# hbdat/cvpr22_cross_modal_pseudo_labeling

Hardware: AMD Instinct MI355X
Metric: images/sec student-teacher train step (COCO 800x1333) (higher is better)
Workload: dtype f32 (bf16x3 split MFMA, fp32 accum); 1 GPU; student_teacher_mask_rcnn_uncertainty.yaml R-50-C4, 2 img/GPU 3x800x1333, fwd+bwd+allreduce+SGD; global_batch=2, parallelism=dp1, losses_finite=True, pipelined=True

## Files before the change

### cvpr22_cross_modal_pseudo_labeling_amd/_C.py

```python
import contextlib
import functools
import ctypes
import threading

import torch

from . import _cpu, _lib

_L = _lib.load()


def _stream():
    return torch._C._cuda_getCurrentRawStream(torch.cuda.current_device())


class _Same:

    def __enter__(self):
        return None

    def __exit__(self, *exc):
        return False


# ... 594 lines not shown
        _lib.check(rc, "match_encode")
    return idx, lab, reg


def rpn_match_encode(gt_boxes, anchors, visibility, high_threshold, low_threshold, allow_low_quality_matches, weights):
    gt_boxes, anchors = _dev(gt_boxes, "gt_boxes"), _dev(anchors, "anchors")
    if not (visibility.is_cuda and visibility.dtype == torch.bool and visibility.shape == (anchors.shape[0],)):
        raise RuntimeError("rpn_match_encode: visibility must be a bool HIP tensor [A]")
    visibility = visibility.contiguous()
    g, a = gt_boxes.shape[0], anchors.shape[0]
    if g == 0:
        raise ValueError("No ground-truth boxes available for one of the images during training")
    labels = torch.empty((a,), dtype=torch.int64, device=anchors.device)
    reg = torch.empty((a, 4), dtype=torch.float32, device=anchors.device)
    scratch = torch.empty((g,), dtype=torch.int32, device=anchors.device)
    wx, wy, ww, wh = weights
    with _on(anchors.device):
        rc = _L.ovis_rpn_match_encode_f32(gt_boxes.data_ptr(), anchors.data_ptr(), visibility.data_ptr(), g, a, high_threshold,
                                          low_threshold, int(bool(allow_low_quality_matches)), wx, wy, ww, wh, scratch.data_ptr(),
                                          labels.data_ptr(), reg.data_ptr(), _stream())
    _lib.check(rc, "rpn_match_encode")
    return labels, reg


def project_masks(masks, gt_index, boxes, resolution):
    if not (masks.is_cuda and masks.dim() == 3 and masks.dtype in (torch.bool, torch.uint8)):
        raise RuntimeError("project_masks: [G,H,W] bool / uint8 HIP tensor expected")
    masks = masks.contiguous()
    boxes = _dev(boxes, "boxes")
    gt_index = gt_index.to(torch.int64).contiguous()
    p = boxes.shape[0]
    out = torch.empty((p, resolution, resolution), dtype=torch.float32, device=boxes.device)
    if p:
        with _on(boxes.device):
            rc = _L.ovis_project_masks_f32(masks.data_ptr(), gt_index.data_ptr(), boxes.data_ptr(), p, masks.shape[1],
                                           masks.shape[2], resolution, int(masks.dtype == torch.bool), out.data_ptr(),
                                           _stream())
        _lib.check(rc, "project_masks")
    return out


def sample_fg_bg(labels, batch_size, max_positives, seed):
    if not labels.is_cuda or labels.dtype != torch.int64 or labels.dim() != 1:
        raise RuntimeError("sample_fg_bg: 1-D int64 HIP tensor expected (the product path has no CPU fallback)")
    labels = labels.contiguous()
    sel = torch.empty((batch_size,), dtype=torch.int64, device=labels.device)
    slots = torch.empty((batch_size,), dtype=torch.int64, device=labels.device)
    counts = torch.empty((2,), dtype=torch.int32, device=labels.device)
    with _on(labels.device):
        rc = _L.ovis_sample_fg_bg(labels.data_ptr(), labels.numel(), int(batch_size), int(max_positives),
                                  int(seed) & 0xFFFFFFFFFFFFFFFF, sel.data_ptr(), slots.data_ptr(), counts.data_ptr(), _stream())
    _lib.check(rc, "sample_fg_bg")
    return sel, slots, counts


def gather_rows(index, boxes_a=None, boxes_b=None, ints_a=None, ints_b=None):
    index = _dev(index, "index", torch.int64)
    n = index.numel()
    srcs = [None if t is None else _dev(t, "boxes", torch.float32) for t in (boxes_a, boxes_b)] + \
           [None if t is None else _dev(t, "ints", torch.int64) for t in (ints_a, ints_b)]
    for t in srcs[:2]:
        if t is not None and (t.dim() != 2 or t.shape[1] != 4):
            raise RuntimeError("gather_rows: float sources must be [P, 4]")
    for t in srcs[2:]:
        if t is not None and t.dim() != 1:
            raise RuntimeError("gather_rows: int64 sources must be [P]")
    outs = [None if t is None else torch.empty((n,) + tuple(t.shape[1:]), dtype=t.dtype, device=t.device) for t in srcs]
    if n:
        with _on(index.device):
            rc = _L.ovis_gather_rows(index.data_ptr(), n, _ptr(srcs[0]), _ptr(outs[0]), _ptr(srcs[1]), _ptr(outs[1]),
                                     _ptr(srcs[2]), _ptr(outs[2]), _ptr(srcs[3]), _ptr(outs[3]), _stream())
        _lib.check(rc, "gather_rows")
    return tuple(outs)


def project_pasted_masks(mask_probs, gt_boxes, gt_index, boxes, image_size, resolution, threshold=0.5):
    mask_probs, gt_boxes, boxes = _dev(mask_probs, "mask_probs"), _dev(gt_boxes, "gt_boxes"), _dev(boxes, "boxes")
    gt_index = _dev(gt_index, "gt_index", torch.int64)
    p = boxes.shape[0]
    out = torch.empty((p, resolution, resolution), dtype=torch.float32, device=boxes.device)
    if p == 0:
        return out
    if mask_probs.dim() != 3 or mask_probs.shape[1] != mask_probs.shape[2] or gt_boxes.shape != (mask_probs.shape[0], 4):
        raise RuntimeError("project_pasted_masks: expected mask_probs [G,M,M] and gt_boxes [G,4]")
    with _on(boxes.device):
        rc = _L.ovis_project_pasted_masks_f32(mask_probs.data_ptr(), gt_boxes.data_ptr(), gt_index.data_ptr(),
                                              boxes.data_ptr(), p, int(image_size[0]), int(image_size[1]),
                                              mask_probs.shape[1], int(resolution), float(threshold), out.data_ptr(), _stream())
    _lib.check(rc, "project_pasted_masks")
    return out


def paste_masks(probs, boxes, image_size, threshold=0.5):
    probs, boxes = _dev(probs, "probs"), _dev(boxes, "boxes")
    if probs.dim() != 3 or probs.shape[1] != probs.shape[2] or boxes.shape != (probs.shape[0], 4):
        raise RuntimeError("paste_masks: expected probs [P,M,M] and boxes [P,4]")
    p, h, w = probs.shape[0], int(image_size[0]), int(image_size[1])
    out = torch.empty((p, h, w), dtype=torch.bool, device=probs.device)
    if p == 0:
        return out
    with _on(probs.device):
        rc = _L.ovis_paste_masks_u8(probs.data_ptr(), boxes.data_ptr(), p, probs.shape[1], h, w, float(threshold),
                                    out.data_ptr(), _stream())
    _lib.check(rc, "paste_masks")
    return out

# ... 1127 lines not shown
```

### cvpr22_cross_modal_pseudo_labeling_amd/csrc/targets.hip

```cpp
#include "ovis_common.h"
#define OVIS_HD __device__ __forceinline__
#include "mask_crop_geom.h"
#include "pasted_geom.h"

namespace {
__global__ __launch_bounds__(256) void match_encode_kernel(const float* __restrict__ gt, const long* __restrict__ gt_labels,
                                                          const float* __restrict__ prop, int G, int P, float high,
                                                          float low, int between_label_mode, float wx, float wy,
                                                          float ww, float wh, long* __restrict__ matched_idx,
                                                          long* __restrict__ labels, float* __restrict__ reg) {
  const int p = blockIdx.x * 256 + threadIdx.x;
  if (p >= P) return;
  const float4 b = *(const float4*)(prop + 4 * p);
  const float area_b = (b.z - b.x + 1.f) * (b.w - b.y + 1.f);
  float best = -1.f;
  int arg = 0;
  for (int g = 0; g < G; ++g) {
    const float4 a = *(const float4*)(gt + 4 * g);
    const float area_a = (a.z - a.x + 1.f) * (a.w - a.y + 1.f);
    const float w = fmaxf(fminf(a.z, b.z) - fmaxf(a.x, b.x) + 1.f, 0.f);
    const float h = fmaxf(fminf(a.w, b.w) - fmaxf(a.y, b.y) + 1.f, 0.f);
    const float inter = w * h;
    const float iou = inter / (area_a + area_b - inter);
    if (iou > best) {
// ... 333 lines not shown
    const int c = (int)(e >> 14);
    if (c == 2) return;
    if (taken(i, e, c)) {
      if (c == 1) pos_slot[pat++] = at;
      sel_idx[at++] = i;
    }
  });
  for (int j = total_sel + tid; j < batch_size; j += kSampThreads) sel_idx[j] = 0;
  for (int j = total_pos + tid; j < batch_size; j += kSampThreads) pos_slot[j] = 0;
  if (tid == 0) {
    counts[0] = total_sel;
    counts[1] = total_pos;
  }
}

__global__ __launch_bounds__(256) void project_pasted_masks_kernel(const float* __restrict__ probs,
                                                                  const float* __restrict__ gt_boxes,
                                                                  const long* __restrict__ gt_index,
                                                                  const float* __restrict__ boxes, int P, int H, int W,
                                                                  int Mp, int M, float thr, float* __restrict__ out) {
  const long i = (long)blockIdx.x * 256 + threadIdx.x;
  const long total = (long)P * M * M;
  if (i >= total) return;
  const int dx = (int)(i % M), dy = (int)((i / M) % M), p = (int)(i / ((long)M * M));
  const MaskCropWindow c = mask_crop_window(*(const float4*)(boxes + 4 * p), W, H);
  const MaskAxisTap ty = mask_axis_tap(dy, c.h, (float)M), tx = mask_axis_tap(dx, c.w, (float)M);
  const float xmin = c.xmin, ymin = c.ymin, y0 = ty.i0, y1 = ty.i1, ly = ty.lam, x0 = tx.i0, x1 = tx.i1, lx = tx.lam;
  const long g = gt_index[p];
  const float4 gb = *(const float4*)(gt_boxes + 4 * g);
  const PastedBox pb = pasted_box(gb, Mp);
  const int4 bx = pb.bx;
  const int bw = pb.bw, bh = pb.bh;
  const float* pr = probs + g * Mp * Mp;
  const int Y0 = (int)(y0 + ymin), Y1 = (int)(y1 + ymin), X0 = (int)(x0 + xmin), X1 = (int)(x1 + xmin);
  const float v00 = pasted_pixel(pr, Mp, bx, bw, bh, thr, H, W, Y0, X0), v01 = pasted_pixel(pr, Mp, bx, bw, bh, thr, H, W, Y0, X1);
  const float v10 = pasted_pixel(pr, Mp, bx, bw, bh, thr, H, W, Y1, X0), v11 = pasted_pixel(pr, Mp, bx, bw, bh, thr, H, W, Y1, X1);
  const float v = (1.f - ly) * ((1.f - lx) * v00 + lx * v01) + ly * ((1.f - lx) * v10 + lx * v11);
  out[i] = v != 0.f ? 1.f : 0.f;
}
__global__ __launch_bounds__(256) void gather_rows_kernel(const long long* __restrict__ index, int n,
                                                         const float4* __restrict__ fa, float4* __restrict__ fa_out,
                                                         const float4* __restrict__ fb, float4* __restrict__ fb_out,
                                                         const long long* __restrict__ ia, long long* __restrict__ ia_out,
                                                         const long long* __restrict__ ib, long long* __restrict__ ib_out) {
  const int i = blockIdx.x * blockDim.x + threadIdx.x;
  if (i >= n) return;
  const long long r = index[i];
  if (fa) fa_out[i] = fa[r];
  if (fb) fb_out[i] = fb[r];
  if (ia) ia_out[i] = ia[r];
  if (ib) ib_out[i] = ib[r];
}

}

extern "C" int ovis_sample_fg_bg(const int64_t* labels, int num, int batch_size, int max_positives, uint64_t seed,
                                 int64_t* selected, int64_t* positive_slots, int32_t* counts, void* stream) {
  if (num < 0 || batch_size <= 0 || max_positives < 0 || max_positives > batch_size) return OVIS_EINVAL;
  if (!selected || !positive_slots || !counts || (num > 0 && !labels)) return OVIS_EINVAL;
  constexpr int kCacheBytes = 150 * 1024;
  if (2L * num + 16 <= kCacheBytes) {
    static bool attr_set = false;
    if (!attr_set) {
      OVIS_HIP_TRY(hipFuncSetAttribute((const void*)sample_fg_bg_kernel<true>, hipFuncAttributeMaxDynamicSharedMemorySize, kCacheBytes));
      attr_set = true;
    }
    const int lds = ((2 * num + 16 + 255) / 256) * 256;
    hipLaunchKernelGGL(sample_fg_bg_kernel<true>, dim3(1), dim3(kSampThreads), lds, (hipStream_t)stream, (const long*)labels, num,
                       batch_size, max_positives, (unsigned long long)seed, (long*)selected, (long*)positive_slots, counts);
  } else {
    hipLaunchKernelGGL(sample_fg_bg_kernel<false>, dim3(1), dim3(kSampThreads), 0, (hipStream_t)stream, (const long*)labels, num,
                       batch_size, max_positives, (unsigned long long)seed, (long*)selected, (long*)positive_slots, counts);
  }
  OVIS_LAUNCH_CHECK();
  return OVIS_OK;
}

extern "C" int ovis_project_pasted_masks_f32(const float* mask_probs, const float* gt_boxes, const int64_t* gt_index,
                                             const float* boxes, int num, int image_height, int image_width,
                                             int prob_resolution, int resolution, float threshold, float* out,
                                             void* stream) {
  if (num < 0 || image_height <= 0 || image_width <= 0 || prob_resolution <= 0 || resolution <= 0) return OVIS_EINVAL;
  if (num == 0) return OVIS_OK;
  if (!mask_probs || !gt_boxes || !gt_index || !boxes || !out) return OVIS_EINVAL;
  if (((uintptr_t)boxes & 15) || ((uintptr_t)gt_boxes & 15)) return OVIS_ERANGE;
  const long total = (long)num * resolution * resolution;
  hipLaunchKernelGGL(project_pasted_masks_kernel, dim3((unsigned)((total + 255) / 256)), dim3(256), 0, (hipStream_t)stream,
                     mask_probs, gt_boxes, (const long*)gt_index, boxes, num, image_height, image_width, prob_resolution,
                     resolution, threshold, out);
  OVIS_LAUNCH_CHECK();
  return OVIS_OK;
}

extern "C" int ovis_match_encode_f32(const float* gt_boxes, const int64_t* gt_labels, const float* proposals,
                                     int num_gt, int num_proposals, float high_threshold, float low_threshold,
                                     int between_keeps_label, float wx, float wy, float ww, float wh,
                                     int64_t* matched_idx, int64_t* labels, float* regression_targets, void* stream) {
  if (num_gt <= 0 || num_proposals < 0) return OVIS_EINVAL;
  if (num_proposals == 0) return OVIS_OK;
  if (!gt_boxes || !gt_labels || !proposals || !matched_idx || !labels) return OVIS_EINVAL;
  if (((uintptr_t)gt_boxes & 15) || ((uintptr_t)proposals & 15) || ((uintptr_t)regression_targets & 15)) return OVIS_ERANGE;
  hipLaunchKernelGGL(match_encode_kernel, dim3((num_proposals + 255) / 256), dim3(256), 0, (hipStream_t)stream, gt_boxes,
                     (const long*)gt_labels, proposals, num_gt, num_proposals, high_threshold, low_threshold,
                     between_keeps_label, wx, wy, ww, wh, (long*)matched_idx, (long*)labels, regression_targets);
  OVIS_LAUNCH_CHECK();
  return OVIS_OK;
// ... 56 lines not shown
```

### cvpr22_cross_modal_pseudo_labeling_amd/engine/trainer.py

```python
import logging
import time

import torch

from . import comm
from .. import _C


def total_loss(loss_dict):
    terms = [v if torch.is_tensor(v) else torch.as_tensor(float(v)) for v in loss_dict.values()]
    if len(terms) < 3 or not all(t.is_cuda for t in terms):
        return sum(terms)
    return torch.stack([t.reshape(()) for t in terms]).sum()


class StepPolicy:

    def __init__(self, accumulation_steps=1, clip_grad_norm_at=-1.0):
        self.accumulation_steps = max(int(accumulation_steps), 1)
        self.clip_grad_norm_at = float(clip_grad_norm_at)
        self.prepare_weights_ahead = True
        self.micro = 0
        self.fresh = True

# ... 28 lines not shown


def train_step(model, optimizer, reducer, images, targets, scheduler=None, policy=None, iteration=None):
    policy = policy or _default_policy(reducer)
    loss_dict = model(images, targets)
    policy.begin(reducer)
    losses = policy.scale(total_loss(loss_dict))
    losses.backward()
    policy.end(reducer, optimizer, scheduler, iteration, model)
    return loss_dict


def _default_policy(reducer):
    pol = getattr(reducer, "_step_policy", None)
    if pol is None:
        pol = reducer._step_policy = StepPolicy()
    return pol


def _record_stream(obj, stream):
    if torch.is_tensor(obj):
        if obj.is_cuda:
            obj.record_stream(stream)
    elif isinstance(obj, dict):
        for v in obj.values():
            _record_stream(v, stream)
    elif isinstance(obj, (list, tuple)):
        for v in obj:
            _record_stream(v, stream)
    elif hasattr(obj, "device_tensors"):
        _record_stream(obj.device_tensors(), stream)


_SIDE_STREAMS = {}


def side_stream(priority):
    key = (torch.cuda.current_device(), priority)
    if key not in _SIDE_STREAMS:
        _SIDE_STREAMS[key] = torch.cuda.Stream(priority=priority)
    return _SIDE_STREAMS[key]


def branch_stream():
    return side_stream(-1)


class PipelinedTrainer:

    def __init__(self, model, optimizer, reducer, scheduler=None, threaded=True, side_priority=-1, policy=None):
        self.model, self.optimizer, self.reducer, self.scheduler = model, optimizer, reducer, scheduler
        self.policy = policy or StepPolicy()
        self.enabled = hasattr(model, "forward_frozen") and torch.cuda.is_available()
        bert = getattr(model, "bert", None)
        if self.enabled and bert is not None and any(p.requires_grad for p in bert.parameters()):
            self.enabled = False
        self.side = side_stream(side_priority) if self.enabled else None
        self.pending = None
        self.threaded = threaded
        self.worker = None
        self.worker_error = None

    def _frozen_on_side(self, images, targets, after_event, device):
        try:
            torch.cuda.set_device(device)
            with torch.cuda.stream(self.side):
                if after_event is not None:
                    self.side.wait_event(after_event)
                with _C.co_scheduled():
                    frozen = self.model.forward_frozen(images, targets)
                done = torch.cuda.Event()
                done.record(self.side)
            self.pending = ((id(images), id(targets)), frozen, done)
        except BaseException as e:
            self.worker_error = e

    def _launch_frozen(self, images, targets, after_event=None, threaded=False):
        device = torch.cuda.current_device()
        if threaded:
            import threading
            self.worker = threading.Thread(target=self._frozen_on_side, args=(images, targets, after_event, device))
            self.worker.start()
        else:
            self._frozen_on_side(images, targets, after_event, device)
            self._check_worker()

    def _check_worker(self):
        if self.worker is not None:
            self.worker.join()
            self.worker = None
        if self.worker_error is not None:
            e, self.worker_error = self.worker_error, None
            raise e

    def step(self, images, targets, next_batch=None, iteration=None):
        if not self.enabled:
            return train_step(self.model, self.optimizer, self.reducer, images, targets, self.scheduler, self.policy, iteration)
        main = torch.cuda.current_stream()
        inputs_ready = torch.cuda.Event()
        inputs_ready.record(main)
        self._check_worker()
        if self.pending is None or self.pending[0] != (id(images), id(targets)):
            self._launch_frozen(images, targets, inputs_ready)
        _, frozen, done = self.pending
        self.pending = None
        main.wait_event(done)
# ... 81 lines not shown
```

### cvpr22_cross_modal_pseudo_labeling_amd/modeling/roi_heads.py

```python
import bisect

import torch
import torch.nn.functional as F
from torch import nn

from .. import _C
from ..layers import (Conv2d, ConvTranspose2d, ROIAlign, linear_mfma, smooth_l1_loss, smooth_l1_picked, stochastic_mask_bce,
                      text_logits, weighted_cross_entropy)
from ..layers.derived import derived
from .backbone import HeadFeatures, ResNetHead
from .box_coder import BoxCoder
from .matcher import BalancedPositiveNegativeSampler, Matcher
from .structures import BoxList, PastedMasks, PolygonMasks, RleMasks, SampledBoxList, box_iou, boxlist_nms, cat_boxlist


def _cat(tensors, dim=0):
    return tensors[0] if len(tensors) == 1 else torch.cat(tensors, dim)


class Pooler(nn.Module):
    def __init__(self, output_size, scales, sampling_ratio):
        super().__init__()
        if len(scales) != 1:
            raise NotImplementedError("single-level pooler only (C4)")
        self.pooler = ROIAlign(output_size, spatial_scale=scales[0], sampling_ratio=sampling_ratio)
        self.output_size = output_size

    @staticmethod
    def convert_to_roi_format(boxes):
        if boxes and all(b.bbox.is_cuda and b.bbox.dtype == torch.float32 for b in boxes):
            return _C.rois_from_boxes([b.bbox for b in boxes])
        parts = []
        for i, b in enumerate(boxes):
            ids = torch.full((len(b), 1), float(i), dtype=b.bbox.dtype, device=b.bbox.device)
            parts.append(torch.cat([ids, b.bbox], dim=1))
        return _cat(parts, 0)

    def forward(self, x, boxes):
        return self.pooler(x[0], self.convert_to_roi_format(boxes))

    def forward_strided_nhwc(self, x, boxes, bin_stride):
        return self.pooler.forward_strided_nhwc(x[0], self.convert_to_roi_format(boxes), bin_stride)


class ResNet50Conv5ROIFeatureExtractor(nn.Module):
    def __init__(self, cfg, head_cfg):
        super().__init__()
        res = head_cfg.POOLER_RESOLUTION
        self.pooler = Pooler((res, res), head_cfg.POOLER_SCALES, head_cfg.POOLER_SAMPLING_RATIO)
        self.head = ResNetHead(cfg)
        self.out_channels = self.head.out_channels

    def forward(self, x, proposals, pooled_only=False):
        return self.forward_rois(x, self.pooler.convert_to_roi_format(proposals), pooled_only=pooled_only)

    def forward_rois(self, x, rois, select=None, pooled_only=False):
        p = self.pooler.pooler
        s = self.head.pooler_stride() if x[0].is_cuda else 0
        if s:
            need_grad = torch.is_grad_enabled() and x[0].requires_grad
            if not need_grad and x[0].shape[1] % 32 == 0 and self.head.pooled_pair_ok():
                ph, pw = p.output_size
                yp, (oh, ow) = _C.roi_align_forward_strided_pair(x[0], rois, p.spatial_scale, ph, pw, p.sampling_ratio, s)
                return self.head.forward_pooled_nhwc(None, yp, (rois.shape[0], oh, ow), select=select, pooled_only=pooled_only)
            return self.head.forward_pooled_nhwc(p.forward_strided_nhwc(x[0], rois, s), select=select, pooled_only=pooled_only)
        return HeadFeatures(self.head(p(x[0], rois)))


class FastRCNNPredictor(nn.Module):

# ... 36 lines not shown
        first = self.emb_pred if self.embedding_based else self.cls_score
        n1 = first.out_features
        n = n1 + self.bbox_pred.out_features
        pad = (-n) % 128 if x.is_cuda else 0

        def concatenated():
            zw, zb = self._zero_rows(pad, x)
            return (torch.cat([first.weight, self.bbox_pred.weight] + ([zw] if pad else []), 0),
                    torch.cat([first.bias, self.bbox_pred.bias] + ([zb] if pad else []), 0))
        w, b = derived((first.weight, first.bias, self.bbox_pred.weight, self.bbox_pred.bias), ("predictor", pad), concatenated)
        y = linear_mfma(x, w, b)
        head, bbox = y[:, :n1], y[:, n1:n]
        if not self.embedding_based:
            return head, bbox
        cls_logit = text_logits(head, self.cls_score if cls_embs is None else cls_embs.to(head.device))
        return cls_logit, bbox

    def _zero_rows(self, pad, x):
        z = getattr(self, "_zero_pad", None)
        if pad and (z is None or z[0].shape[0] != pad or z[0].device != x.device):
            z = (x.new_zeros((pad, self.bbox_pred.in_features)), x.new_zeros((pad,)))
            self._zero_pad = z
        return z if pad else (None, None)

    def embed(self, x):
        if not self.embedding_based:
            raise RuntimeError("FastRCNNPredictor.embed: MODEL.ROI_BOX_HEAD.EMBEDDING_BASED is False -- there is no embedding "
                               "projection to align with text")
        return linear_mfma(self.pooled(x), self.emb_pred.weight, self.emb_pred.bias)

    def set_class_embeddings(self, embs):
        if not self.embedding_based:
            raise RuntimeError("set_class_embeddings: MODEL.ROI_BOX_HEAD.EMBEDDING_BASED is False -- the classifier is a "
                               "learned Linear over NUM_CLASSES")
        self.num_classes = embs.shape[0]
        self.cls_score = embs.to(self.emb_pred.weight.device)


class FastRCNNLossComputation:
    def __init__(self, cfg):
        rh = cfg.MODEL.ROI_HEADS
        self.matcher = Matcher(rh.FG_IOU_THRESHOLD, rh.BG_IOU_THRESHOLD, allow_low_quality_matches=False)
        self.sampler = BalancedPositiveNegativeSampler(rh.BATCH_SIZE_PER_IMAGE, rh.POSITIVE_FRACTION)
        self.box_coder = BoxCoder(weights=rh.BBOX_REG_WEIGHTS)
        self.cls_agnostic_bbox_reg = cfg.MODEL.CLS_AGNOSTIC_BBOX_REG
        self.bg_weight = cfg.MODEL.ROI_BOX_HEAD.LOSS_WEIGHT_BACKGROUND
        self.generator = None
        self.device_sampler = True

    def subsample(self, proposals, targets):
        return self.subsample_many([(proposals, targets)])[0]

    def subsample_many(self, groups):
        if not all(p.bbox.is_cuda for props, _ in groups for p in props) or self.matcher.allow_low_quality_matches \
                or not self.device_sampler:
            return [self._subsample_tensor_ops(props, tgts) for props, tgts in groups]
        pending = []
        for props, tgts in groups:
            for prop, tgt in zip(props, tgts):
                idx, labels, reg = _C.match_encode(tgt.bbox, tgt.get_field("labels"), prop.bbox, self.matcher.high_threshold,
                                                   self.matcher.low_threshold, self.box_coder.weights)
                sel, slots, counts = self.sampler.sample_device(labels, self.generator)
                pending.append((prop, idx, labels, reg, sel, slots, counts))
        cnt = torch.stack([p[-1] for p in pending]).tolist() if pending else []
        out, k = [], 0
        for props, _ in groups:
            group = []
            for _p in props:
                prop, idx, labels, reg, sel, slots, _c = pending[k]
                n, npos = cnt[k]
                k += 1
                bbox_s, reg_s, labels_s, idx_s = _C.gather_rows(sel[:n], prop.bbox, reg, labels, idx)
                b = BoxList(bbox_s, prop.size)
                b.add_field("labels", labels_s)
                b.add_field("regression_targets", reg_s)
                b.add_field("matched_gt", idx_s)
                group.append(SampledBoxList(b, slots[:npos]))
            out.append(group)
        self._proposals = out[-1]
        return out

    def _subsample_tensor_ops(self, proposals, targets):
        out = []
        labels_all = []
        for prop, tgt in zip(proposals, targets):
            if prop.bbox.is_cuda and not self.matcher.allow_low_quality_matches:
                idx, labels, reg = _C.match_encode(tgt.bbox, tgt.get_field("labels"), prop.bbox,
                                                   self.matcher.high_threshold, self.matcher.low_threshold,
                                                   self.box_coder.weights)
            else:
                matched = self.matcher(box_iou(tgt.bbox, prop.bbox))
                idx = matched.clamp(min=0)
                labels = tgt.get_field("labels")[idx].to(torch.int64)
                labels[matched == Matcher.BELOW_LOW_THRESHOLD] = 0
                labels[matched == Matcher.BETWEEN_THRESHOLDS] = -1
                reg = self.box_coder.encode(tgt.bbox[idx], prop.bbox)
            prop.add_field("labels", labels)
            prop.add_field("regression_targets", reg)
            prop.add_field("matched_gt", idx)
            labels_all.append(labels)
        pos, neg = self.sampler(labels_all, generator=self.generator)
        for prop, p, n in zip(proposals, pos, neg):
            out.append(SampledBoxList(prop[torch.nonzero(p | n).squeeze(1)]))
        self._proposals = out
        return out

    def __call__(self, class_logits, box_regression, proposals=None):
        if proposals is None:
            proposals = self._proposals
        labels = _cat([p.get_field("labels") for p in proposals], 0)
        reg_targets = _cat([p.get_field("regression_targets") for p in proposals], 0)
        pos = positives_index(proposals)
        if pos is None:
            pos = torch.nonzero(labels > 0).squeeze(1)
        if box_regression.is_cuda and labels.numel():
            box_loss = smooth_l1_picked(box_regression, reg_targets, pos, None if self.cls_agnostic_bbox_reg else labels, 4,
                                        1.0, labels.numel())
        else:
            if self.cls_agnostic_bbox_reg:
                picked = box_regression.index_select(0, pos)[:, 4:8]
            else:
                map_inds = 4 * labels[pos][:, None] + torch.tensor([0, 1, 2, 3], device=class_logits.device)
                picked = box_regression[pos[:, None], map_inds]
            box_loss = smooth_l1_loss(picked, reg_targets.index_select(0, pos), size_average=False, beta=1) / labels.numel()
        cls_loss = weighted_cross_entropy(class_logits, labels, self.bg_weight)
        return cls_loss, box_loss


def positives_index(proposals):
    parts, off = [], 0
    for p in proposals:
        if not isinstance(p, SampledBoxList) or p.pos_index is None:
            return None
# ... 479 lines not shown
        self.avg_uncertain = "N/A"

    def forward(self, features, proposals, targets=None, compute_uncertain=False, eps=None):
        if self.training:
            sel = positives_index(proposals)
            if sel is not None:
                proposals = [positive_proposals(p) for p in proposals]
            else:
                positive_inds = [p.get_field("labels") > 0 for p in proposals]
                proposals = [p[i] for p, i in zip(proposals, positive_inds)]
                sel = _cat(positive_inds, 0)
        if self.training and self.share:
            fl = features.permute(0, 2, 3, 1) if features.dim() == 4 else None
            if fl is not None and fl.is_contiguous() and not features.is_contiguous():
                x = fl[sel].permute(0, 3, 1, 2)
            else:
                x = features[sel]
        else:
            x = self.feature_extractor(features, proposals).maps
        if self.training:
            return x, proposals, dict(loss_mask=self.fused_training_loss(x, proposals, targets, compute_uncertain, eps))
        if compute_uncertain:
            mask_logits, scale = self.predictor(x, True, eps=eps)
            self.log, self.avg_uncertain = scale.max(), scale.mean()
        else:
            mask_logits = self.predictor(x)
        prob = mask_logits.sigmoid()
        if self.cls_agnostic_mask:
            prob = prob[:, 1][:, None]
        else:
            labels = _cat([b.get_field("labels") for b in proposals], 0)
            prob = prob[torch.arange(prob.shape[0], device=prob.device), labels][:, None]
        results = []
        for p, b in zip(prob.split([len(b) for b in proposals], 0), proposals):
            out = b.copy_with_fields(b.fields())
            out.add_field("mask", p if self.masker is None else self.masker(p, b))
            results.append(out)
        return x, results, {}

    def fused_training_loss(self, x, proposals, targets, compute_uncertain=False, eps=None):
        mu, sigma = self.predictor.forward_parts(x)
        if compute_uncertain and sigma is not None:
            self.log, self.avg_uncertain = sigma.max(), sigma.mean()
            if eps is None:
                eps = torch.randn((1, *mu.shape), device=mu.device, dtype=mu.dtype)
            else:
                eps = eps[:, : mu.shape[0]].to(mu.device)
            return self.loss_evaluator.fused(proposals, mu, sigma, eps, targets)
        return self.loss_evaluator.fused(proposals, mu, None, None, targets)


class CombinedROIHeads(nn.ModuleDict):
    batch_branches = True

    def __init__(self, cfg, in_channels, is_teacher=False):
        heads = [("box", ROIBoxHead(cfg, in_channels, is_teacher))]
        if cfg.MODEL.MASK_ON:
            heads.append(("mask", ROIMaskHead(cfg, in_channels)))
        super().__init__(heads)
        self.cfg = cfg
        self.mask_on = cfg.MODEL.MASK_ON
        if self.mask_on and cfg.MODEL.ROI_MASK_HEAD.SHARE_BOX_FEATURE_EXTRACTOR:
            self.mask.feature_extractor = self.box.feature_extractor

    def branches_batchable(self, feat):
        return (self.training and feat.is_cuda and (not self.mask_on or (self.mask.share and self.mask.cls_agnostic_mask))
                and self.batch_branches)

    def forward_branches(self, feat, branches):
        box = self.box
        with torch.no_grad():
            sampled = box.loss_evaluator.subsample_many([(br["proposals"], br["targets"]) for br in branches])
        rois = _C.rois_from_boxes([p.bbox for props in sampled for p in props],
                                  [img for br in branches for img in br["image_ids"]])
        sel_pos = positives_index([p for props in sampled for p in props]) if self.mask_on else None
        x, pooled, handed = box.feature_extractor.forward_rois([feat], rois, select=sel_pos)
        pooled = box.predictor.pooled(pooled if pooled is not None else x)
        counts = [sum(len(p) for p in props) for props in sampled]
        out, off = [], 0
        for br, props, cnt in zip(branches, sampled, counts):
            class_logits, box_regression = box.predictor(pooled[off:off + cnt], br["cls_embs"])
            lc, lb = box.loss_evaluator(class_logits, box_regression, props)
            out.append(dict(loss_classifier=lc, loss_box_reg=lb))
            off += cnt
        if self.mask_on:
            mask = self.mask
            sel = sel_pos
            if sel is not None:
                pos_all = [[positive_proposals(p) for p in props] for props in sampled]
            else:
                pos_masks = [[p.get_field("labels") > 0 for p in props] for props in sampled]
                sel = _cat([m for ms in pos_masks for m in ms], 0)
                pos_all = [[p[m] for p, m in zip(props, ms)] for props, ms in zip(sampled, pos_masks)]
            fl = x.permute(0, 2, 3, 1)
            if handed is not None and handed[0] is sel:
                xs = handed[1].view(sel.numel(), x.shape[2], x.shape[3], x.shape[1]).permute(0, 3, 1, 2)
            else:
                xs = fl[sel].permute(0, 3, 1, 2) if (fl.is_contiguous() and not x.is_contiguous()) else x[sel]
            off = 0
            for br, pos_props, losses in zip(branches, pos_all, out):
                k = sum(len(p) for p in pos_props)
                losses["loss_mask"] = mask.fused_training_loss(xs[off:off + k], pos_props, br["targets"],
                                                               br.get("compute_uncertain", False), br.get("eps"))
                off += k
        return out

    def forward(self, features, proposals, targets=None, bbox_only=False, compute_uncertain=False, eps=None,
                is_eval_func=False, cls_embs=None, unfiltered=False):
        losses, package_x = {}, {}
        gt_boxes = self.cfg.MODEL.GT_BOX_EVAL and is_eval_func and not self.training
        if gt_boxes:
            device = features[0].device if isinstance(features, (list, tuple)) else features.device
            proposals = []
            for t in targets:
                det = t.copy_with_fields(["labels"])
                det.add_field("objectness", t.get_field("labels") * 0.0 + 1.0)
                proposals.append(det.to(device))
        x, detections, loss_box = self.box(features, proposals, targets, cls_embs, unfiltered=unfiltered)
        if gt_boxes:
            for det, tar in zip(detections, targets):
                assert len(det) == len(tar), "GT_BOX_EVAL keeps one detection per ground-truth box"
        package_x["bbox"] = x
        losses.update(loss_box)
        if self.mask_on and not bbox_only:
            mask_features = features
            if self.training and self.cfg.MODEL.ROI_MASK_HEAD.SHARE_BOX_FEATURE_EXTRACTOR:
                mask_features = x
            x, detections, loss_mask = self.mask(mask_features, detections, targets, compute_uncertain, eps=eps)
            package_x["mask"] = x
            losses.update(loss_mask)
        return package_x, detections, losses
```

### include/ovis_hip.h

```cpp
#ifndef OVIS_HIP_H_
#define OVIS_HIP_H_

#include <stddef.h>
#include <stdint.h>

#ifdef __cplusplus
extern "C" {
#endif

#define OVIS_OK 0
#define OVIS_EINVAL (-1)
#define OVIS_ENOSPC (-2)
#define OVIS_ERANGE (-3)

const char* ovis_version(void);

int ovis_roi_align_forward_f32(const float* input, const float* rois, float* output,
                               int num_rois, int batch, int channels, int height,
                               int width, int pooled_h, int pooled_w,
                               float spatial_scale, int sampling_ratio, void* stream);

size_t ovis_roi_align_forward_workspace_bytes(int num_rois, int height, int width);
int ovis_roi_align_forward_mfma_supported(int height, int width, int pooled_h, int pooled_w);
int ovis_roi_align_forward_ws_f32(const float* input, const float* rois, float* output,
// ... 132 lines not shown

int ovis_im2col_pair(const void* src_pair, void* dst_pair, long num, int height, int width,
                     int channels, int kh, int kw, void* stream);

int ovis_split_gemm_pair_gated_ws(const void* a_pair, long a_row_bytes, const void* b_pair, long b_row_bytes,
                                  float* c, long ldc, void* c_pair, long c_pair_row_bytes, const void* gate_pair,
                                  long gate_row_bytes, long m, int n, int channels, int taps_h, int taps_w,
                                  int height, int width, int flip, void* workspace, size_t workspace_bytes,
                                  int config, void* stream);

int ovis_split_gemm_pair_rp_gated(const void* a_pair, long a_row_bytes, const void* b_pair, long b_row_bytes, float* c,
                                  long ldc, void* c_pair, long c_pair_row_bytes, const void* residual_pair,
                                  long residual_pair_row_bytes, const void* gate_pair, long gate_row_bytes, long m, int n,
                                  int channels, int config, void* stream);

int ovis_im2col_nchw_pair_f32(const float* src, void* dst_pair, int num, int channels, int height, int width,
                              int kh, int kw, int stride, int pad, int k_padded, void* stream);

size_t ovis_split_gemm_pair_workspace_bytes(long m, int n, int channels, int channels2, int taps_h, int taps_w,
                                            int width);
size_t ovis_split_gemm_pair_workspace_bytes_ex(long m, int n, int channels, int channels2, int taps_h, int taps_w,
                                               int width, int config);
int ovis_split_gemm_pair(const void* a_pair, long a_row_bytes, const void* a2_pair, long a2_row_bytes,
                         const void* b_pair, long b_row_bytes, float* c, long ldc, void* c_pair,
                         long c_pair_row_bytes, const float* bias, const float* residual, long ldr, long m,
                         int n, int channels, int channels2, int taps_h, int taps_w, int height, int width,
                         int flip, int relu, void* workspace, size_t workspace_bytes, int config, void* stream);
int ovis_split_gemm_pair_rp(const void* a_pair, long a_row_bytes, const void* b_pair, long b_row_bytes, float* c, long ldc,
                            void* c_pair, long c_pair_row_bytes, const float* bias, const void* residual_pair,
                            long residual_pair_row_bytes, long m, int n, int channels, int relu, void* workspace,
                            size_t workspace_bytes, int config, void* stream);

int ovis_split_gemm_tn_slices(long m, int n, int channels, int taps);
int ovis_split_gemm_tn_map_slices(long m, int n, int channels, int taps_h, int taps_w, int height, int width);
int ovis_split_gemm_pair_tn(const void* g_pair, long g_row_bytes, const void* x_pair, long x_row_bytes,
                            float* c_slabs, int slices, long m, int n, int channels, int taps_h,
                            int taps_w, int height, int width, void* stream);

int ovis_match_encode_f32(const float* gt_boxes, const int64_t* gt_labels, const float* proposals, int num_gt,
                          int num_proposals, float high_threshold, float low_threshold, int between_keeps_label,
                          float wx, float wy, float ww, float wh, int64_t* matched_idx, int64_t* labels,
                          float* regression_targets, void* stream);
int ovis_rpn_match_encode_f32(const float* gt_boxes, const float* anchors, const uint8_t* visibility, int num_gt,
                              int num_anchors, float high_threshold, float low_threshold, int allow_low_quality_matches,
                              float wx, float wy, float ww, float wh, uint32_t* best_per_gt_scratch, int64_t* labels,
                              float* regression_targets, void* stream);
int ovis_project_masks_f32(const uint8_t* masks, const int64_t* gt_index, const float* boxes, int num, int height,
                           int width, int resolution, int masks_are_bool, float* out, void* stream);
int ovis_sample_fg_bg(const int64_t* labels, int num, int batch_size, int max_positives, uint64_t seed,
                      int64_t* selected, int64_t* positive_slots, int32_t* counts, void* stream);
int ovis_project_pasted_masks_f32(const float* mask_probs, const float* gt_boxes, const int64_t* gt_index,
                                  const float* boxes, int num, int image_height, int image_width, int prob_resolution,
                                  int resolution, float threshold, float* out, void* stream);
int ovis_paste_masks_u8(const float* mask_probs, const float* boxes, int num, int prob_resolution, int image_height,
                        int image_width, float threshold, uint8_t* out, void* stream);
int ovis_pasted_rle_count(const float* mask_probs, const float* boxes, const int32_t* image_sizes, int num,
                          int prob_resolution, float threshold, int32_t* num_runs, void* stream);
int ovis_pasted_rle_runs(const float* mask_probs, const float* boxes, const int32_t* image_sizes, int num,
                         int prob_resolution, float threshold, const int64_t* run_offsets, int32_t* runs,
                         int32_t* num_chars, void* stream);
int ovis_pasted_rle_string(const int32_t* runs, const int64_t* run_offsets, const int64_t* char_offsets, int num,
                           uint8_t* out, void* stream);
int ovis_render_instances_u8(const uint8_t* image, int height, int width, const float* maps, const float* boxes,
                             int num_layers, int map_resolution, const int32_t* kinds, const float* params,
                             const float* colors, float alpha, const uint8_t* outline_colors, int outline_thickness,
                             uint8_t* out, void* stream);
int ovis_gather_rows(const int64_t* index, int num, const float* boxes_a, float* boxes_a_out, const float* boxes_b,
                     float* boxes_b_out, const int64_t* ints_a, int64_t* ints_a_out, const int64_t* ints_b,
                     int64_t* ints_b_out, void* stream);

int ovis_gemm_f32(const float* A, long a_row_stride, long a_k_stride, const float* B,
                  long b_row_stride, long b_k_stride, const float* bias, float* C,
                  long c_row_stride, int M, int N, int K, void* stream);

int ovis_gemm_ex_f32(const float* A, long a_row_stride, long a_k_stride, const float* B,
                     long b_row_stride, long b_k_stride, const float* bias, int bias_per_row,
                     float alpha, int accumulate, float* C, long c_row_stride, int M, int N, int K,
                     void* stream);

size_t ovis_gemm_f32_workspace_bytes(int M, int N, int K);
int ovis_gemm_ex_ws_f32(const float* A, long a_row_stride, long a_k_stride, const float* B,
                        long b_row_stride, long b_k_stride, const float* bias, int bias_per_row,
                        float alpha, int accumulate, float* C, long c_row_stride, int M, int N, int K,
                        void* workspace, size_t workspace_bytes, void* stream);

int ovis_region_noun_align_f32(const float* region_emb, const float* noun_emb, float* raw_scores,
                               float* sigmoid_scores, int64_t* best_region, int num_regions,
                               int num_nouns, int dim, void* stream);

int ovis_weighted_ce_fwd_bwd_f32(const float* logits, const int64_t* labels, float bg_weight,
                                 float* loss, float* dlogits, float* row_scratch, int num_rows,
                                 int num_classes, void* stream);
int ovis_mask_bce_stochastic_fwd_bwd_f32(const float* mu, const float* sigma, const float* eps,
                                         const int64_t* pos_index, const float* targets, float* loss,
                                         float* dmu, float* dsigma, float* row_scratch, int num_rois,
                                         int num_pos, int num_channels, int mask_pixels, int channel,
                                         void* stream);
int ovis_mask_bce_stochastic_classes_fwd_bwd_f32(const float* mu, const float* sigma, const float* eps,
                                                 const int64_t* pos_index, const int64_t* channels,
                                                 const float* targets, float* loss, float* dmu, float* dsigma,
                                                 float* row_scratch, int num_rois, int num_pos,
                                                 int num_channels, int mask_pixels, void* stream);

int ovis_deform_im2col_f32(const float* input, const float* offset, const float* mask, float* columns,
                           int num_images, int channels, int height, int width, int kernel_h,
                           int kernel_w, int pad_h, int pad_w, int stride_h, int stride_w,
// ... 108 lines not shown
```

Baseline: 60.86 images/sec.

## Deduplicate sampled RoIs shared between student branches before box/mask heads

Adds a single-block HIP kernel that unions the sampled RoIs of two branches on the same images. Boxes are matched by hash plus exact compare, and the kernel builds index maps so duplicate RoIs are pooled and run through the box feature extractor only once. The trainer turns this on for the student heads, and predictor and mask inputs are then gathered through index_select. Savings depend on how many sampled proposals the two branches share. The cost is an extra serial kernel, O(n^2) matching, and gather ops, and gradients now flow through shared rows.

```diff
diff --git a/cvpr22_cross_modal_pseudo_labeling_amd/_C.py b/cvpr22_cross_modal_pseudo_labeling_amd/_C.py
--- a/cvpr22_cross_modal_pseudo_labeling_amd/_C.py
+++ b/cvpr22_cross_modal_pseudo_labeling_amd/_C.py
@@ -670,6 +670,45 @@
                                   int(seed) & 0xFFFFFFFFFFFFFFFF, sel.data_ptr(), slots.data_ptr(), counts.data_ptr(), _stream())
     _lib.check(rc, "sample_fg_bg")
     return sel, slots, counts
+
+
+BRANCH_ROI_UNION_MAX_IMAGES = _lib.OVIS_BOX_DECODE_MAX_IMAGES
+
+
+def branch_roi_union(branch0, branch1, image_ids=None):
+    n = len(branch0)
+    if n == 0 or len(branch1) != n:
+        raise RuntimeError("branch_roi_union: the same, non-zero number of images expected in both branches")
+    cols = []
+    for name, branch in (("branch0", branch0), ("branch1", branch1)):
+        boxes = [_dev(b[0], f"{name} boxes") for b in branch]
+        sel = [_dev(b[1], f"{name} selected", torch.int64) for b in branch]
+        slots = [_dev(b[2], f"{name} positive_slots", torch.int64) for b in branch]
+        counts = [_dev(b[3], f"{name} counts", torch.int32) for b in branch]
+        batch = sel[0].numel()
+        if any(b.dim() != 2 or b.shape[1] != 4 for b in boxes) or any(c.numel() != 2 for c in counts) \
+                or any(s.numel() != batch for s in sel + slots) or batch == 0:
+            raise RuntimeError(f"branch_roi_union: {name}: [P, 4] boxes, equally long selected / positive_slots and [2] counts expected")
+        cols.append((boxes, sel, slots, counts, batch))
+    dev = cols[0][0][0].device
+    b0, b1 = cols[0][4], cols[1][4]
+    rows = -(-n * (b0 + b1) // 32) * 32
+    rois = torch.empty((rows, 5), dtype=torch.float32, device=dev)
+    i64 = torch.empty((n * (2 * b0 + 3 * b1),), dtype=torch.int64, device=dev)
+    map1, positive_rows, slots0, slots1 = i64.split([n * b1, n * (b0 + b1), n * b0, n * b1])
+    i32 = torch.empty((b0 + 2 * n,), dtype=torch.int32, device=dev)
+
+    def table(tensors, ctype=ctypes.c_void_p):
+        return (ctype * n)(*[t.data_ptr() if t.numel() else None for t in tensors])
+    args = []
+    for boxes, sel, slots, counts, _ in cols:
+        args += [table(boxes), (ctypes.c_int32 * n)(*[b.shape[0] for b in boxes]), table(sel), table(slots), table(counts)]
+    ids = None if image_ids is None else (ctypes.c_int32 * n)(*[int(i) for i in image_ids])
+    with _on(dev):
+        rc = _L.ovis_branch_roi_union(*args, ids, n, b0, b1, rois.data_ptr(), rows, map1.data_ptr(), positive_rows.data_ptr(),
+                                      slots0.data_ptr(), slots1.data_ptr(), i32.data_ptr(), i32[b0:].data_ptr(), _stream())
+    _lib.check(rc, "branch_roi_union")
+    return rois, map1, positive_rows, slots0, slots1, i32[b0:].view(n, 2)
 
 
 def gather_rows(index, boxes_a=None, boxes_b=None, ints_a=None, ints_b=None):
diff --git a/cvpr22_cross_modal_pseudo_labeling_amd/csrc/targets.hip b/cvpr22_cross_modal_pseudo_labeling_amd/csrc/targets.hip
--- a/cvpr22_cross_modal_pseudo_labeling_amd/csrc/targets.hip
+++ b/cvpr22_cross_modal_pseudo_labeling_amd/csrc/targets.hip
@@ -409,6 +409,256 @@
   if (ib) ib_out[i] = ib[r];
 }
 
+constexpr int kUnionStage = 512;
+
+struct UnionImages {
+  int count;
+  int image_id[OVIS_BOX_DECODE_MAX_IMAGES];
+  int num[2][OVIS_BOX_DECODE_MAX_IMAGES];
+  const float* boxes[2][OVIS_BOX_DECODE_MAX_IMAGES];
+  const long* selected[2][OVIS_BOX_DECODE_MAX_IMAGES];
+  const long* slots[2][OVIS_BOX_DECODE_MAX_IMAGES];
+  const int* counts[2][OVIS_BOX_DECODE_MAX_IMAGES];
+};
+
+__device__ __forceinline__ unsigned union_hash(uint4 b) {
+  return b.x ^ ((b.y << 8) | (b.y >> 24)) ^ ((b.z << 16) | (b.z >> 16)) ^ ((b.w << 24) | (b.w >> 8));
+}
+
+__device__ __forceinline__ uint4 union_box(const float* __restrict__ boxes, const long* __restrict__ selected, int r, int P) {
+  long s = selected[r];
+  s = s < 0 ? 0 : (s >= P ? P - 1 : s);
+  return *(const uint4*)(boxes + 4 * s);
+}
+
+__device__ __forceinline__ void union_write_roi(float* __restrict__ rois, long row, int id, uint4 b) {
+  float* o = rois + 5 * row;
+  o[0] = (float)id;
+  o[1] = __uint_as_float(b.x);
+  o[2] = __uint_as_float(b.y);
+  o[3] = __uint_as_float(b.z);
+  o[4] = __uint_as_float(b.w);
+}
+
+__device__ int union_first_equal(const float* __restrict__ boxes, const long* __restrict__ selected, int n, int P, uint4 mine,
+                                 bool active, uint4* sbox, unsigned* shash) {
+  const unsigned mh = union_hash(mine);
+  int first = n;
+  for (int s = 0; s < n; s += kUnionStage) {
+    const int cnt = min(kUnionStage, n - s);
+    __syncthreads();
+    for (int r = threadIdx.x; r < kUnionStage; r += kSampThreads) {
+      if (r < cnt) {
+        const uint4 b = union_box(boxes, selected, s + r, P);
+        sbox[r] = b;
+        shash[r] = union_hash(b);
+      } else {
+        shash[r] = 0u;
+      }
+    }
+    __syncthreads();
+    if (active && first == n) {
+      for (int g = 0; g < cnt && first == n; g += 4) {
+        const uint4 h = *(const uint4*)(shash + g);
+        if (h.x == mh || h.y == mh || h.z == mh || h.w == mh) {
+          const unsigned hh[4] = {h.x, h.y, h.z, h.w};
+#pragma unroll
+          for (int u = 0; u < 4; ++u) {
+            const int r = g + u;
+            if (first == n && r < cnt && hh[u] == mh) {
+              const uint4 b = sbox[r];
+              if (b.x == mine.x && b.y == mine.y && b.z == mine.z && b.w == mine.w) first = s + r;
+            }
+          }
+        }
+      }
+    }
+  }
+  return first;
+}
+
+__global__ __launch_bounds__(kSampThreads) void branch_roi_union_kernel(UnionImages in, int batch0, int batch1,
+                                                                        float* __restrict__ rois, int rois_rows,
+                                                                        long* __restrict__ map1, long* __restrict__ pos_rows,
+                                                                        long* __restrict__ slots0_out,
+                                                                        long* __restrict__ slots1_out, int* __restrict__ mark,
+                                                                        int* __restrict__ out_counts) {
+  __shared__ uint4 sbox[kUnionStage];
+  __shared__ __attribute__((aligned(16))) unsigned shash[kUnionStage];
+  __shared__ int sh[kSampThreads / 64];
+  __shared__ int ns[2][OVIS_BOX_DECODE_MAX_IMAGES], ps[2][OVIS_BOX_DECODE_MAX_IMAGES];
+  __shared__ int new_rows[OVIS_BOX_DECODE_MAX_IMAGES], len_a[OVIS_BOX_DECODE_MAX_IMAGES];
+  const int tid = threadIdx.x;
+  if (tid < 2 * in.count) {
+    const int b = tid & 1, img = tid >> 1;
+    const int cap = b ? batch1 : batch0;
+    int n = in.counts[b][img][0], p = in.counts[b][img][1];
+    n = in.num[b][img] > 0 ? max(0, min(n, cap)) : 0;
+    ns[b][img] = n;
+    ps[b][img] = max(0, min(p, n));
+  }
+  __syncthreads();
+  int total0 = 0;
+  for (int img = 0; img < in.count; ++img) total0 += ns[0][img];
+  int base0 = 0, base1 = 0, new_base = 0, a_base = 0, ps0 = 0, ps1 = 0;
+  for (int img = 0; img < in.count; ++img) {
+    const int n0 = ns[0][img], n1 = ns[1][img], p0 = ps[0][img], p1 = ps[1][img], id = in.image_id[img];
+    const int P0 = in.num[0][img], P1 = in.num[1][img];
+    const float* boxes0 = in.boxes[0][img];
+    const float* boxes1 = in.boxes[1][img];
+    const long *sel0 = in.selected[0][img], *sel1 = in.selected[1][img];
+    const long *slots0 = in.slots[0][img], *slots1 = in.slots[1][img];
+    for (int r = tid; r < n0; r += kSampThreads) union_write_roi(rois, base0 + r, id, union_box(boxes0, sel0, r, P0));
+    int img_new = 0;
+    for (int jb = 0; jb < n1; jb += kSampThreads) {
+      const int j = jb + tid;
+      const bool active = j < n1;
+      const uint4 mine = active ? union_box(boxes1, sel1, j, P1) : make_uint4(0u, 0u, 0u, 0u);
+      const int i = union_first_equal(boxes0, sel0, n0, P0, mine, active, sbox, shash);
+      const int upto = min(n1, jb + kSampThreads);
+      const int j_first = union_first_equal(boxes1, sel1, upto, P1, mine, active, sbox, shash);
+      const bool matched = active && i < n0 && j_first == j;
+      int tot;
+      const int k = block_exscan(active && !matched ? 1 : 0, sh, &tot);
+      if (active) {
+        const long u = matched ? (long)(base0 + i) : (long)(total0 + new_base + img_new + k);
+        map1[base1 + j] = u;
+        if (!matched) union_write_roi(rois, u, id, mine);
+      }
+      img_new += tot;
+    }
+    for (int r = tid; r < n0; r += kSampThreads) mark[r] = 0;
+    __syncthreads();
+    for (int t = tid; t < p0; t += kSampThreads) {
+      const long s = slots0[t];
+      if (s >= 0 && s < n0) mark[s] = 1;
+    }
+    for (int t = tid; t < p1; t += kSampThreads) {
+      const long j = slots1[t];
+      if (j >= 0 && j < n1) {
+        const long u = map1[base1 + j];
+        if (u < total0) mark[u - base0] = 1;
+      }
+    }
+    __syncthreads();
+    int la = 0;
+    for (int rb = 0; rb < n0; rb += kSampThreads) {
+      const int r = rb + tid;
+      const bool f = r < n0 && mark[r] != 0;
+      int tot;
+      const int k = block_exscan(f ? 1 : 0, sh, &tot);
+      if (f) {
+        pos_rows[a_base + la + k] = base0 + r;
+        mark[r] = a_base + la + k + 1;
+      }
+      la += tot;
+    }
+    __syncthreads();
+    for (int t = tid; t < p0; t += kSampThreads) {
+      const long s = slots0[t];
+      slots0_out[ps0 + t] = (s >= 0 && s < n0) ? mark[s] - 1 : 0;
+    }
+    for (int t = tid; t < p1; t += kSampThreads) {
+      const long j = slots1[t];
+      long at = 0;
+      if (j >= 0 && j < n1) {
+        const long u = map1[base1 + j];
+        if (u < total0) at = mark[u - base0] - 1;
+      }
+      slots1_out[ps1 + t] = at;
+    }
+    if (tid == 0) {
+      new_rows[img] = img_new;
+      len_a[img] = la;
+    }
+    __syncthreads();
+    base0 += n0;
+    base1 += n1;
+    new_base += img_new;
+    a_base += la;
+    ps0 += p0;
+    ps1 += p1;
+  }
+  int b_base = a_base;
+  base1 = 0;
+  ps1 = 0;
+  for (int img = 0; img < in.count; ++img) {
+    const int n1 = ns[1][img], p1 = ps[1][img];
+    const long* slots1 = in.slots[1][img];
+    int lb = 0;
+    for (int tb = 0; tb < p1; tb += kSampThreads) {
+      const int t = tb + tid;
+      long u = 0;
+      bool f = false;
+      if (t < p1) {
+        const long j = slots1[t];
+        if (j >= 0 && j < n1) {
+          u = map1[base1 + j];
+          f = u >= total0;
+        }
+      }
+      int tot;
+      const int k = block_exscan(f ? 1 : 0, sh, &tot);
+      if (f) {
+        pos_rows[b_base + lb + k] = u;
+        slots1_out[ps1 + t] = b_base + lb + k;
+      }
+      lb += tot;
+    }
+    if (tid == 0) {
+      out_counts[2 * img] = new_rows[img];
+      out_counts[2 * img + 1] = len_a[img] + lb;
+    }
+    b_base += lb;
+    base1 += n1;
+    ps1 += p1;
+  }
+  const int rows = total0 + new_base;
+  __syncthreads();
+  for (int r = rows + tid; r < rois_rows; r += kSampThreads) {
+#pragma unroll
+    for (int c = 0; c < 5; ++c) rois[5 * (long)r + c] = rows > 0 ? rois[5 * (long)(rows - 1) + c] : (c == 0 ? (float)in.image_id[0] : 0.f);
+  }
+}
+
+}
+
+extern "C" int ovis_branch_roi_union(const float* const* boxes0, const int32_t* num0, const int64_t* const* selected0,
+                                     const int64_t* const* positive_slots0, const int32_t* const* counts0,
+                                     const float* const* boxes1, const int32_t* num1, const int64_t* const* selected1,
+                                     const int64_t* const* positive_slots1, const int32_t* const* counts1,
+                                     const int32_t* image_ids, int num_images, int batch0, int batch1, float* rois,
+                                     int rois_rows, int64_t* map1, int64_t* positive_rows, int64_t* slots0, int64_t* slots1,
+                                     int32_t* workspace, int32_t* out_counts, void* stream) {
+  if (num_images <= 0 || batch0 <= 0 || batch1 <= 0) return OVIS_EINVAL;
+  if (num_images > OVIS_BOX_DECODE_MAX_IMAGES || (long)num_images * ((long)batch0 + batch1) > (1L << 26)) return OVIS_ERANGE;
+  if (rois_rows < (long)num_images * ((long)batch0 + batch1)) return OVIS_ENOSPC;
+  if (!boxes0 || !num0 || !selected0 || !positive_slots0 || !counts0 || !boxes1 || !num1 || !selected1 || !positive_slots1 ||
+      !counts1 || !rois || !map1 || !positive_rows || !slots0 || !slots1 || !workspace || !out_counts)
+    return OVIS_EINVAL;
+  UnionImages in;
+  in.count = num_images;
+  for (int i = 0; i < num_images; ++i) {
+    const float* bx[2] = {boxes0[i], boxes1[i]};
+    const int nb[2] = {num0[i], num1[i]};
+    const int64_t* se[2] = {selected0[i], selected1[i]};
+    const int64_t* sl[2] = {positive_slots0[i], positive_slots1[i]};
+    const int32_t* ct[2] = {counts0[i], counts1[i]};
+    for (int b = 0; b < 2; ++b) {
+      if (nb[b] < 0 || (nb[b] > 0 && !bx[b]) || !se[b] || !sl[b] || !ct[b]) return OVIS_EINVAL;
+      if ((uintptr_t)bx[b] & 15) return OVIS_ERANGE;
+      in.num[b][i] = nb[b];
+      in.boxes[b][i] = bx[b];
+      in.selected[b][i] = (const long*)se[b];
+      in.slots[b][i] = (const long*)sl[b];
+      in.counts[b][i] = ct[b];
+    }
+    in.image_id[i] = image_ids ? image_ids[i] : i;
+  }
+  hipLaunchKernelGGL(branch_roi_union_kernel, dim3(1), dim3(kSampThreads), 0, (hipStream_t)stream, in, batch0, batch1, rois,
+                     rois_rows, (long*)map1, (long*)positive_rows, (long*)slots0, (long*)slots1, workspace, out_counts);
+  OVIS_LAUNCH_CHECK();
+  return OVIS_OK;
 }
 
 extern "C" int ovis_sample_fg_bg(const int64_t* labels, int num, int batch_size, int max_positives, uint64_t seed,
diff --git a/cvpr22_cross_modal_pseudo_labeling_amd/engine/trainer.py b/cvpr22_cross_modal_pseudo_labeling_amd/engine/trainer.py
--- a/cvpr22_cross_modal_pseudo_labeling_amd/engine/trainer.py
+++ b/cvpr22_cross_modal_pseudo_labeling_amd/engine/trainer.py
@@ -104,6 +104,9 @@
         self.model, self.optimizer, self.reducer, self.scheduler = model, optimizer, reducer, scheduler
         self.policy = policy or StepPolicy()
         self.enabled = hasattr(model, "forward_frozen") and torch.cuda.is_available()
+        student_heads = getattr(model, "roi_heads_student", None)
+        if hasattr(student_heads, "share_branch_rois"):
+            student_heads.share_branch_rois = True
         bert = getattr(model, "bert", None)
         if self.enabled and bert is not None and any(p.requires_grad for p in bert.parameters()):
             self.enabled = False
diff --git a/cvpr22_cross_modal_pseudo_labeling_amd/modeling/roi_heads.py b/cvpr22_cross_modal_pseudo_labeling_amd/modeling/roi_heads.py
--- a/cvpr22_cross_modal_pseudo_labeling_amd/modeling/roi_heads.py
+++ b/cvpr22_cross_modal_pseudo_labeling_amd/modeling/roi_heads.py
@@ -1,4 +1,5 @@
 import bisect
+from collections import namedtuple
 
 import torch
 import torch.nn.functional as F
@@ -16,6 +17,9 @@
 
 def _cat(tensors, dim=0):
     return tensors[0] if len(tensors) == 1 else torch.cat(tensors, dim)
+
+
+BranchRoiUnion = namedtuple("BranchRoiUnion", "rois rows0 map1 positive_rows slots0 slots1")
 
 
 class Pooler(nn.Module):
@@ -158,9 +162,12 @@
         return self.subsample_many([(proposals, targets)])[0]
 
     def subsample_many(self, groups):
+        return self.subsample_branches(groups)[0]
+
+    def subsample_branches(self, groups, union_image_ids=None):
         if not all(p.bbox.is_cuda for props, _ in groups for p in props) or self.matcher.allow_low_quality_matches \
                 or not self.device_sampler:
-            return [self._subsample_tensor_ops(props, tgts) for props, tgts in groups]
+            return [self._subsample_tensor_ops(props, tgts) for props, tgts in groups], None
         pending = []
         for props, tgts in groups:
             for prop, tgt in zip(props, tgts):
@@ -168,7 +175,22 @@
                                                    self.matcher.low_threshold, self.box_coder.weights)
                 sel, slots, counts = self.sampler.sample_device(labels, self.generator)
                 pending.append((prop, idx, labels, reg, sel, slots, counts))
-        cnt = torch.stack([p[-1] for p in pending]).tolist() if pending else []
+        union, count_rows = None, [p[-1] for p in pending]
+        n_img = len(groups[0][0]) if groups else 0
+        if union_image_ids is not None and len(groups) == 2 and len(groups[1][0]) == n_img == len(union_image_ids) \
+                and 0 < n_img <= _C.BRANCH_ROI_UNION_MAX_IMAGES:
+            union = _C.branch_roi_union(*([(p[0].bbox, p[4], p[5], p[6]) for p in pending[b * n_img:(b + 1) * n_img]]
+                                          for b in (0, 1)), union_image_ids)
+            count_rows = count_rows + list(union[5].unbind(0))
+        cnt = torch.stack(count_rows).tolist() if pending else []
+        if union is not None:
+            rois, map1, positive_rows, slots0, slots1, _ = union
+            own, extra = cnt[:len(pending)], cnt[len(pending):]
+            rows0 = sum(c[0] for c in own[:n_img])
+            rows = rows0 + sum(e[0] for e in extra)
+            union = BranchRoiUnion(rois[:-(-rows // 32) * 32], rows0, map1[:sum(c[0] for c in own[n_img:])],
+                                   positive_rows[:sum(e[1] for e in extra)], slots0[:sum(c[1] for c in own[:n_img])],
+                                   slots1[:sum(c[1] for c in own[n_img:])])
         out, k = [], 0
         for props, _ in groups:
             group = []
@@ -184,7 +206,7 @@
                 group.append(SampledBoxList(b, slots[:npos]))
             out.append(group)
         self._proposals = out[-1]
-        return out
+        return out, union
 
     def _subsample_tensor_ops(self, proposals, targets):
         out = []
@@ -770,6 +792,7 @@
 
 class CombinedROIHeads(nn.ModuleDict):
     batch_branches = True
+    share_branch_rois = False
 
     def __init__(self, cfg, in_channels, is_teacher=False):
         heads = [("box", ROIBoxHead(cfg, in_channels, is_teacher))]
@@ -787,17 +810,28 @@
 
     def forward_branches(self, feat, branches):
         box = self.box
+        share = (self.share_branch_rois and len(branches) == 2
+                 and list(branches[0]["image_ids"]) == list(branches[1]["image_ids"]))
         with torch.no_grad():
-            sampled = box.loss_evaluator.subsample_many([(br["proposals"], br["targets"]) for br in branches])
-        rois = _C.rois_from_boxes([p.bbox for props in sampled for p in props],
-                                  [img for br in branches for img in br["image_ids"]])
-        sel_pos = positives_index([p for props in sampled for p in props]) if self.mask_on else None
+            sampled, union = box.loss_evaluator.subsample_branches([(br["proposals"], br["targets"]) for br in branches],
+                                                                   list(branches[0]["image_ids"]) if share else None)
+        if union is not None:
+            rois = union.rois
+            sel_pos = union.positive_rows if self.mask_on else None
+        else:
+            rois = _C.rois_from_boxes([p.bbox for props in sampled for p in props],
+                                      [img for br in branches for img in br["image_ids"]])
+            sel_pos = positives_index([p for props in sampled for p in props]) if self.mask_on else None
         x, pooled, handed = box.feature_extractor.forward_rois([feat], rois, select=sel_pos)
         pooled = box.predictor.pooled(pooled if pooled is not None else x)
         counts = [sum(len(p) for p in props) for props in sampled]
         out, off = [], 0
-        for br, props, cnt in zip(branches, sampled, counts):
-            class_logits, box_regression = box.predictor(pooled[off:off + cnt], br["cls_embs"])
+        for b, (br, props, cnt) in enumerate(zip(branches, sampled, counts)):
+            if union is None:
+                rows = pooled[off:off + cnt]
+            else:
+                rows = pooled[:cnt] if b == 0 else pooled.index_select(0, union.map1)
+            class_logits, box_regression = box.predictor(rows, br["cls_embs"])
             lc, lb = box.loss_evaluator(class_logits, box_regression, props)
             out.append(dict(loss_classifier=lc, loss_box_reg=lb))
             off += cnt
@@ -816,9 +850,10 @@
             else:
                 xs = fl[sel].permute(0, 3, 1, 2) if (fl.is_contiguous() and not x.is_contiguous()) else x[sel]
             off = 0
-            for br, pos_props, losses in zip(branches, pos_all, out):
+            for b, (br, pos_props, losses) in enumerate(zip(branches, pos_all, out)):
                 k = sum(len(p) for p in pos_props)
-                losses["loss_mask"] = mask.fused_training_loss(xs[off:off + k], pos_props, br["targets"],
+                xb = xs[off:off + k] if union is None else xs.index_select(0, union.slots1 if b else union.slots0)
+                losses["loss_mask"] = mask.fused_training_loss(xb, pos_props, br["targets"],
                                                                br.get("compute_uncertain", False), br.get("eps"))
                 off += k
         return out
diff --git a/include/ovis_hip.h b/include/ovis_hip.h
--- a/include/ovis_hip.h
+++ b/include/ovis_hip.h
@@ -208,6 +208,13 @@
 int ovis_project_pasted_masks_f32(const float* mask_probs, const float* gt_boxes, const int64_t* gt_index,
                                   const float* boxes, int num, int image_height, int image_width, int prob_resolution,
                                   int resolution, float threshold, float* out, void* stream);
+int ovis_branch_roi_union(const float* const* boxes0, const int32_t* num0, const int64_t* const* selected0,
+                          const int64_t* const* positive_slots0, const int32_t* const* counts0,
+                          const float* const* boxes1, const int32_t* num1, const int64_t* const* selected1,
+                          const int64_t* const* positive_slots1, const int32_t* const* counts1, const int32_t* image_ids,
+                          int num_images, int batch0, int batch1, float* rois, int rois_rows, int64_t* map1,
+                          int64_t* positive_rows, int64_t* slots0, int64_t* slots1, int32_t* workspace,
+                          int32_t* out_counts, void* stream);
 int ovis_paste_masks_u8(const float* mask_probs, const float* boxes, int num, int prob_resolution, int image_height,
                         int image_width, float threshold, uint8_t* out, void* stream);
 int ovis_pasted_rle_count(const float* mask_probs, const float* boxes, const int32_t* image_sizes, int num,
```

Result: faster. 65.99 images/sec, median of 6 (+8.4%).
